# ncarraz/ESRGANplus

Measured on AMD Instinct MI355X. Metric: HR megapixels/sec (x4 SR) RRDBNet forward (fwd+bwd: the fwd_bwd object of this line), higher is better.
Workload: dtype f16; 1 GPU; RRDBNet x4 (23 RRDB, nf=64, gc=32) fp16 forward-only, batch 16 of 128x128 LR tiles per GPU -> 512x512 HR (BASELINE configs[1]); global_batch=16, parallelism=dp1 (independent tiles, no collective), weights=synthetic default-init seed 0

## Files before the change

### esrganplus_amd/_lib.py

```python
import ctypes as C
import os
import threading

import torch

_HERE = os.path.dirname(os.path.abspath(__file__))
LIB_PATH = os.environ.get('ESR_LIB_PATH', os.path.join(_HERE, 'libesrgan_hip.so'))

ESR_F16, ESR_F32 = 0, 1
ACT_NONE, ACT_LRELU, ACT_RELU = 0, 1, 2
NOISE_OFF, NOISE_PHILOX, NOISE_EXPLICIT = 0, 1, 2
OP_CONV, OP_PACK, OP_LAYOUT, OP_NOISE_FILL, OP_WGRAD, OP_BN, OP_POOL, OP_LINEAR, OP_UNPERMUTE, OP_PACK_BATCH = 1, 2, 3, 4, 5, 6, 7, 8, 9, 10
OP_RDB_CHAIN, OP_FRAG_GATHER, OP_RDB_WGRAD, OP_RDB_CHAIN_BWD = 11, 12, 13, 14
BN_STATS, BN_FINALIZE, BN_APPLY, BN_BWD_REDUCE, BN_BWD_FINAL, BN_BWD_APPLY, BN_RESTAT, BN_FIN_APPLY = 0, 1, 2, 3, 4, 5, 6, 7
NO_LAYER = 0xFFFFFFFF
POOL_FWD, POOL_BWD, POOL_SHUFFLE, POOL_UNSHUFFLE = 0, 1, 2, 3


class esr_g32(C.Structure):
    _fields_ = [('ptr', C.c_void_p), ('batch_stride', C.c_int64), ('group_stride', C.c_int64),
                ('wp', C.c_int32), ('ngroups', C.c_int32)]


class esr_conv(C.Structure):
    _fields_ = [('dtype', C.c_int32), ('ks', C.c_int32), ('stride', C.c_int32),
                ('upsample', C.c_int32), ('B', C.c_int32), ('H', C.c_int32), ('W', C.c_int32),
                ('cin_groups', C.c_int32), ('cout_blocks', C.c_int32),
                ('in_', esr_g32), ('out', esr_g32),
                ('w', C.c_void_p), ('bias', C.c_void_p), ('w1x1', C.c_void_p),
                ('n1x1_groups', C.c_int32), ('act', C.c_int32),
                ('aux_out', esr_g32),
                ('alpha', C.c_float), ('res1', esr_g32),
                ('beta', C.c_float), ('res2', esr_g32),
                ('noise_mode', C.c_int32), ('sigma', C.c_float), ('seed', C.c_uint64),
                ('layer1', C.c_uint32), ('layer2', C.c_uint32),
                ('z1', esr_g32), ('z2', esr_g32), ('mask', esr_g32), ('out2', esr_g32),
                ('nchw_out_c', C.c_int32), ('nchw_out', C.c_void_p),
                ('debug_flags', C.c_int32), ('mask_cb_begin', C.c_int32), ('gamma', C.c_float),
                ('layer3', C.c_uint32), ('z3', esr_g32), ('out3', esr_g32),
                ('mask_act', C.c_int32), ('_pad2', C.c_int32), ('seed_dev', C.c_void_p),
                ('ksplit', C.c_int32), ('stat_groups', C.c_int32), ('stat_C', C.c_int32), ('_pad3', C.c_int32),
                ('split_ws', C.c_void_p), ('stat_sums', C.c_void_p)]


class esr_pack(C.Structure):
    _fields_ = [('src', C.c_void_p), ('dst', C.c_void_p), ('cout', C.c_int32), ('cin', C.c_int32),
                ('ks', C.c_int32), ('dtype', C.c_int32), ('transpose_flip', C.c_int32),
                ('sum_dst', C.c_int32), ('sum_src', C.c_int32), ('sum_count', C.c_int32),
                ('ups_dgrad', C.c_int32),
                ('gather', C.c_int32), ('dst_cout', C.c_int32), ('dst_chunk0', C.c_int32),
                ('dst_nchunks', C.c_int32), ('src_co0', C.c_int32), ('src_ks', C.c_int32),
                ('scale', C.c_float), ('ups_fwd', C.c_int32), ('fold_co0', C.c_int32), ('one_t', C.c_int32)]


class esr_wgrad(C.Structure):
    _fields_ = [('dtype', C.c_int32), ('ks', C.c_int32), ('stride', C.c_int32),
                ('upsample', C.c_int32), ('B', C.c_int32), ('H', C.c_int32), ('W', C.c_int32),
                ('cout', C.c_int32), ('cin', C.c_int32), ('g', esr_g32), ('in_', esr_g32),
                ('dw', C.c_void_p), ('dbias', C.c_void_p), ('scale', C.c_float), ('tap_major', C.c_int32),
                ('partial', C.c_void_p), ('partial_elems', C.c_int64)]


class esr_layout(C.Structure):
    _fields_ = [('dtype', C.c_int32), ('to_g32', C.c_int32), ('B', C.c_int32), ('C', C.c_int32),
                ('H', C.c_int32), ('W', C.c_int32), ('nchw', C.c_void_p), ('g32', esr_g32),
                ('use_affine', C.c_int32), ('mean_c', C.c_float * 4), ('inv_std_c', C.c_float * 4),
                ('accumulate', C.c_int32), ('_pad', C.c_int32)]


class esr_noise_fill(C.Structure):
    _fields_ = [('dst', C.c_void_p), ('B', C.c_int32), ('C', C.c_int32), ('H', C.c_int32),
                ('W', C.c_int32), ('seed', C.c_uint64), ('layer', C.c_uint32)]


class esr_bn(C.Structure):
    _fields_ = [('dtype', C.c_int32), ('mode', C.c_int32), ('B', C.c_int32), ('C', C.c_int32),
                ('H', C.c_int32), ('W', C.c_int32), ('training', C.c_int32), ('act', C.c_int32),
                ('momentum', C.c_float), ('eps', C.c_float),
                ('x', esr_g32), ('y', esr_g32), ('g', esr_g32), ('gx', esr_g32),
                ('sums', C.c_void_p), ('mean', C.c_void_p), ('invstd', C.c_void_p),
                ('gamma', C.c_void_p), ('beta', C.c_void_p), ('running_mean', C.c_void_p),
                ('running_var', C.c_void_p), ('dgamma', C.c_void_p), ('dbeta', C.c_void_p),
                ('groups', C.c_int32), ('_pad', C.c_int32), ('num_batches_tracked', C.c_void_p)]


class esr_pool(C.Structure):
    _fields_ = [('dtype', C.c_int32), ('mode', C.c_int32), ('B', C.c_int32), ('C', C.c_int32),
                ('H', C.c_int32), ('W', C.c_int32), ('relu_mask', C.c_int32), ('_pad', C.c_int32),
                ('x', esr_g32), ('y', esr_g32), ('g', esr_g32), ('gx', esr_g32)]


class esr_linear(C.Structure):
    _fields_ = [('mode', C.c_int32), ('B', C.c_int32), ('I', C.c_int32), ('O', C.c_int32),
                ('act', C.c_int32), ('in_act', C.c_int32),
                ('x', C.c_void_p), ('w', C.c_void_p), ('b', C.c_void_p), ('y', C.c_void_p),
# ... 70 lines not shown
                ('band_rows', C.c_int32), ('band_margin', C.c_int32), ('img_H', C.c_int32), ('_pad3', C.c_int32)]


class esr_l1_loss(C.Structure):
    _fields_ = [('a', C.c_void_p), ('b', C.c_void_p), ('grad_a', C.c_void_p), ('loss', C.c_void_p),
                ('scratch', C.c_void_p), ('n', C.c_int64), ('weight', C.c_float), ('grad_scale', C.c_float),
                ('grad_scale_dev', C.c_void_p)]


class esr_ragan_loss(C.Structure):
    _fields_ = [('x', C.c_void_p), ('y', C.c_void_p), ('grad_x', C.c_void_p), ('grad_y', C.c_void_p),
                ('loss', C.c_void_p), ('mean_x', C.c_void_p), ('mean_y', C.c_void_p),
                ('bce_x', C.c_void_p), ('bce_y', C.c_void_p), ('n', C.c_int32),
                ('tx', C.c_float), ('ty', C.c_float), ('weight', C.c_float),
                ('mode', C.c_int32), ('grad_scale', C.c_float), ('sums', C.c_void_p), ('ext', C.c_void_p),
                ('grad_scale_dev', C.c_void_p)]


class esr_img_metrics(C.Structure):
    _fields_ = [('sr', C.c_void_p), ('hr', C.c_void_p), ('C', C.c_int32), ('H', C.c_int32), ('W', C.c_int32),
                ('crop', C.c_int32), ('y_only', C.c_int32), ('_pad', C.c_int32), ('lo', C.c_float), ('hi', C.c_float),
                ('img_sr', C.c_void_p), ('img_hr', C.c_void_p), ('y_sr', C.c_void_p), ('y_hr', C.c_void_p),
                ('out', C.c_void_p), ('win', C.c_double * 11)]


class esr_frag_gather(C.Structure):
    _fields_ = [('src_off', C.c_void_p), ('src_base', C.c_void_p), ('dst', C.c_void_p), ('n', C.c_int64),
                ('piece_bytes', C.c_int32), ('_pad', C.c_int32)]


class esr_rdb_wgrad_block(C.Structure):
    _fields_ = [('in_', esr_g32), ('q', esr_g32), ('dw', C.c_void_p * 6), ('db', C.c_void_p * 6)]


class esr_rdb_wgrad(C.Structure):
    _fields_ = [('dtype', C.c_int32), ('B', C.c_int32), ('H', C.c_int32), ('W', C.c_int32),
                ('n_blocks', C.c_int32), ('tap_major', C.c_int32), ('scale5', C.c_float), ('scale', C.c_float),
                ('blocks', C.c_void_p), ('partial', C.c_void_p), ('partial_elems', C.c_int64),
                ('max_workgroups', C.c_int32), ('_pad', C.c_int32)]


class _op_union(C.Union):
    _fields_ = [('conv', esr_conv), ('pack', esr_pack), ('layout', esr_layout),
                ('noise_fill', esr_noise_fill), ('wgrad', esr_wgrad), ('bn', esr_bn),
                ('pool', esr_pool), ('linear', esr_linear), ('unpermute', esr_unpermute),
                ('pack_batch', esr_pack_batch), ('rdb_chain', esr_rdb_chain), ('frag_gather', esr_frag_gather),
                ('rdb_wgrad', esr_rdb_wgrad)]


class esr_op(C.Structure):
    _fields_ = [('kind', C.c_int32), ('flags', C.c_int32), ('u', _op_union)]


EXPORTS = ['esr_packed_weight_bytes', 'esr_g32_dims', 'esr_conv_forward', 'esr_pack_conv_weights',
           'esr_convert_layout', 'esr_fill_noise', 'esr_conv_wgrad', 'esr_conv_wgrad_multi', 'esr_batchnorm', 'esr_maxpool2',
           'esr_linear_op', 'esr_grad_unpermute', 'esr_adam_step', 'esr_amp_step', 'esr_resample_axis', 'esr_pack_conv_weights_batch', 'esr_pack_pieces',
           'esr_run_ops', 'esr_run_ops_timed', 'esr_graph_create', 'esr_graph_launch', 'esr_graph_destroy', 'esr_last_error',
           'esr_abi_version', 'esr_sizeof_op', 'esr_rdb_forward', 'esr_rdb_workspace_bytes', 'esr_rdb_weight_stream_bytes',
           'esr_rdb_max_tiles_per_image', 'esr_gather_fragments', 'esr_image_metrics', 'esr_wgrad_workspace_elems',
           'esr_l1_loss_forward', 'esr_ragan_loss_forward', 'esr_rdb_wgrad_run', 'esr_rdb_wgrad_workspace_elems', 'esr_rdb_backward',
           'esr_rdb_mask_bytes', 'esr_rdb_check_abort', 'esr_debug_hold_cus', 'esr_debug_device_alias', 'esr_debug_chain_order_waits',
           'esr_debug_mfma_probe', 'esr_debug_rdb_wgrad_follow']

_lib = None
_lock = threading.Lock()


class HipExtensionError(RuntimeError):
    pass


def lib():
    global _lib
    if _lib is not None:
        return _lib
    with _lock:
        if _lib is not None:
            return _lib
        if not os.path.exists(LIB_PATH):
            raise HipExtensionError(
                'esrganplus_amd: %s not found — build it with `python -c "import __graft_entry__ as g; '
                'g.build()"` (hipcc --offload-arch=gfx950). There is no CPU/eager fallback.' % LIB_PATH)
        L = C.CDLL(LIB_PATH)
        for name in EXPORTS:
            if not hasattr(L, name):
                raise HipExtensionError('libesrgan_hip.so lacks symbol ' + name)
        L.esr_last_error.restype = C.c_char_p
        L.esr_sizeof_op.restype = C.c_size_t
        L.esr_pack_pieces.restype = C.c_int64
        L.esr_pack_pieces.argtypes = [C.POINTER(esr_pack)]
        L.esr_packed_weight_bytes.restype = C.c_size_t
        L.esr_packed_weight_bytes.argtypes = [C.c_int32] * 4
        L.esr_g32_dims.restype = None
        L.esr_g32_dims.argtypes = [C.c_int32, C.c_int32, C.POINTER(C.c_int32), C.POINTER(C.c_int32)]
        L.esr_run_ops.argtypes = [C.c_void_p, C.c_int32, C.c_void_p]
        L.esr_run_ops_timed.argtypes = [C.c_void_p, C.c_int32, C.c_void_p, C.c_void_p]
        L.esr_graph_create.argtypes = [C.c_void_p, C.c_int32, C.POINTER(C.c_void_p)]
        L.esr_graph_launch.argtypes = [C.c_void_p, C.c_void_p]
        L.esr_graph_destroy.argtypes = [C.c_void_p]
        L.esr_conv_wgrad_multi.argtypes = [C.POINTER(esr_wgrad), C.c_int32, C.c_void_p]
        L.esr_wgrad_workspace_elems.restype = C.c_int64
        L.esr_wgrad_workspace_elems.argtypes = [C.c_void_p, C.c_int32]
        L.esr_rdb_workspace_bytes.restype = C.c_size_t
        L.esr_rdb_workspace_bytes.argtypes = [C.c_int32] * 3
        L.esr_rdb_weight_stream_bytes.restype = C.c_size_t
        L.esr_rdb_weight_stream_bytes.argtypes = [C.c_int32]
        L.esr_rdb_mask_bytes.restype = C.c_size_t
        L.esr_rdb_mask_bytes.argtypes = [C.c_int32] * 3
        L.esr_debug_chain_order_waits.restype = C.c_uint64
        L.esr_debug_device_alias.argtypes = [C.c_int32]
        L.esr_rdb_wgrad_workspace_elems.restype = C.c_int64
        L.esr_rdb_wgrad_workspace_elems.argtypes = [C.c_int32] * 4
        for name, st in (('esr_conv_forward', esr_conv), ('esr_pack_conv_weights', esr_pack),
                         ('esr_convert_layout', esr_layout), ('esr_fill_noise', esr_noise_fill),
                         ('esr_conv_wgrad', esr_wgrad), ('esr_batchnorm', esr_bn),
                         ('esr_maxpool2', esr_pool), ('esr_linear_op', esr_linear),
                         ('esr_grad_unpermute', esr_unpermute), ('esr_adam_step', esr_adam), ('esr_amp_step', esr_amp), ('esr_resample_axis', esr_resample),
                         ('esr_pack_conv_weights_batch', esr_pack_batch), ('esr_rdb_forward', esr_rdb_chain),
                         ('esr_gather_fragments', esr_frag_gather), ('esr_image_metrics', esr_img_metrics),
                         ('esr_l1_loss_forward', esr_l1_loss), ('esr_ragan_loss_forward', esr_ragan_loss),
                         ('esr_rdb_wgrad_run', esr_rdb_wgrad), ('esr_rdb_backward', esr_rdb_chain)):
            getattr(L, name).argtypes = [C.POINTER(st), C.c_void_p]
        if L.esr_sizeof_op() != C.sizeof(esr_op):
            raise HipExtensionError('ABI mismatch: sizeof(esr_op) C=%d ctypes=%d'
                                    % (L.esr_sizeof_op(), C.sizeof(esr_op)))
        _lib = L
    return _lib


def check(rc, what=''):
    if rc != 0:
        raise HipExtensionError('%s failed (%d): %s' % (what or 'libesrgan_hip', rc,
                                                        lib().esr_last_error().decode()))


def g32_dims(h, w):
    hp, wp = C.c_int32(), C.c_int32()
    lib().esr_g32_dims(h, w, C.byref(hp), C.byref(wp))
    return hp.value, wp.value


def packed_weight_bytes(cout, cin, ks, dtype):
    return lib().esr_packed_weight_bytes(cout, cin, ks, dtype)


OPF_SIDE = 1
OPF_FOLLOW = 4
OPF_SIDE_FREE = 2


class OpList:

    def __init__(self):
        self.ops = []
        self._arr = None
        self.keep = []

    def add_conv(self, conv):
        o = esr_op()
        o.kind = OP_CONV
        o.u.conv = conv
        self.ops.append(o)
        self._arr = None
        self.drop_graph()
        return len(self.ops) - 1

# ... 73 lines not shown
```

### esrganplus_amd/csrc/api.hip

```cpp
#include <stdarg.h>
#include <stdio.h>
#include <stdlib.h>
#include <mutex>

#include "common.h"

namespace {
thread_local char g_err[512] = "";
}

void esr_set_error(const char* fmt, ...) {
  va_list ap;
  va_start(ap, fmt);
  vsnprintf(g_err, sizeof(g_err), fmt, ap);
  va_end(ap);
}

int esr_check_launch(const char* what) {
  const hipError_t e = hipGetLastError();
  if (e != hipSuccess) {
    esr_set_error("%s: %s", what, hipGetErrorString(e));
    return ESR_ERR_LAUNCH;
  }
  return ESR_OK;
// ... 21 lines not shown
namespace {
constexpr int NFREE = 3;
struct SideState { std::mutex mu; hipStream_t owner; hipStream_t stream; hipEvent_t fork[2], join[2]; hipStream_t xs[NFREE]; hipEvent_t xfork, xjoin[NFREE]; SideState* next; };
SideState* side_state(hipStream_t owner) {
  static std::mutex mu;
  static SideState* per_dev[64] = {};
  const int dev = esr_bookkeeping_device();
  static const bool per_stream = [] { const char* e = getenv("ESR_SIDE_PER_STREAM"); return e && atoi(e) != 0; }();
  if (!per_stream) owner = nullptr;
  std::lock_guard<std::mutex> lk(mu);
  for (SideState* s = per_dev[dev]; s; s = s->next)
    if (s->owner == owner) return s;
  SideState* s = new SideState();
  s->owner = owner;
  bool ok = hipStreamCreateWithFlags(&s->stream, hipStreamNonBlocking) == hipSuccess;
  for (int k = 0; k < 2 && ok; ++k)
    ok = hipEventCreateWithFlags(&s->fork[k], hipEventDisableTiming) == hipSuccess &&
         hipEventCreateWithFlags(&s->join[k], hipEventDisableTiming) == hipSuccess;
  ok = ok && hipEventCreateWithFlags(&s->xfork, hipEventDisableTiming) == hipSuccess;
  for (int k = 0; k < NFREE && ok; ++k)
    ok = hipStreamCreateWithFlags(&s->xs[k], hipStreamNonBlocking) == hipSuccess &&
         hipEventCreateWithFlags(&s->xjoin[k], hipEventDisableTiming) == hipSuccess;
  if (!ok) { esr_set_error("side stream: creation failed"); delete s; return nullptr; }
  s->next = per_dev[dev];
  per_dev[dev] = s;
  return s;
}
}

int esr_rdb_backward_with_follower(const esr_rdb_chain* ch, const esr_rdb_wgrad* wg, hipStream_t stream, hipStream_t side, hipEvent_t fork);

constexpr int ESR_WGRAD_RUN_MAX = 24;

extern "C" int esr_run_ops(const esr_op* ops, int32_t n, esr_stream_t stream) {
  if (!ops || n < 0) { esr_set_error("esr_run_ops: invalid arguments"); return ESR_ERR_INVALID; }
  if (esr_rdb_check_abort()) {
    esr_set_error("esr_run_ops: an earlier fused-chain launch aborted (a tile waited > 1 s for its neighbours: CUs held by other work?) — its results are invalid");
    return ESR_ERR_LAUNCH;
  }
  int nside = 0;
  bool joined = true;
  int nfree = 0;
  auto join_free = [&]() -> int {
    if (nfree > 0) {
      SideState* ss = side_state((hipStream_t)stream);
      for (int q = 0; q < NFREE && q < nfree; ++q) ESR_HIP(hipStreamWaitEvent((hipStream_t)stream, ss->xjoin[q], 0));
      nfree = 0;
    }
    return ESR_OK;
  };
  for (int i = 0; i < n; ++i) {
    int rc;
    switch (ops[i].kind) {
      case ESR_OP_CONV: rc = esr_conv_forward(&ops[i].u.conv, stream); break;
      case ESR_OP_PACK: rc = esr_pack_conv_weights(&ops[i].u.pack, stream); break;
      case ESR_OP_LAYOUT: rc = esr_convert_layout(&ops[i].u.layout, stream); break;
      case ESR_OP_NOISE_FILL: rc = esr_fill_noise(&ops[i].u.noise_fill, stream); break;
      case ESR_OP_WGRAD: {
        const int side = ops[i].flags & ESR_OPF_SIDE;
        int m = 1;
        while (i + m < n && m < ESR_WGRAD_RUN_MAX && ops[i + m].kind == ESR_OP_WGRAD && (ops[i + m].flags & ESR_OPF_SIDE) == side) ++m;
        esr_wgrad run[ESR_WGRAD_RUN_MAX];
        for (int k = 0; k < m; ++k) run[k] = ops[i + k].u.wgrad;
        if (!side) {
          rc = m == 1 ? esr_conv_wgrad(&run[0], stream) : esr_conv_wgrad_multi(run, m, stream);
        } else if (ops[i].flags & ESR_OPF_SIDE_FREE) {
          SideState* ss = side_state((hipStream_t)stream);
          if (!ss) return ESR_ERR_LAUNCH;
          const int q = nfree % NFREE;
          {
            std::lock_guard<std::mutex> lk(ss->mu);
            ESR_HIP(hipEventRecord(ss->xfork, (hipStream_t)stream));
            ESR_HIP(hipStreamWaitEvent(ss->xs[q], ss->xfork, 0));
          }
          rc = esr_conv_wgrad_multi(run, m, (esr_stream_t)ss->xs[q]);
          ESR_HIP(hipEventRecord(ss->xjoin[q], ss->xs[q]));
          ++nfree;
        } else {
          SideState* ss = side_state((hipStream_t)stream);
          if (!ss) return ESR_ERR_LAUNCH;
          hipStream_t main_st = (hipStream_t)stream;
          if (nside > 0) ESR_HIP(hipStreamWaitEvent(main_st, ss->join[(nside - 1) & 1], 0));
          {
            std::lock_guard<std::mutex> lk(ss->mu);
            ESR_HIP(hipEventRecord(ss->fork[nside & 1], main_st));
            ESR_HIP(hipStreamWaitEvent(ss->stream, ss->fork[nside & 1], 0));
          }
          rc = esr_conv_wgrad_multi(run, m, (esr_stream_t)ss->stream);
          ESR_HIP(hipEventRecord(ss->join[nside & 1], ss->stream));
          ++nside;
          joined = false;
        }
        if (rc == ESR_OK) i += m - 1;
        break;
      }
      case ESR_OP_BN: rc = esr_batchnorm(&ops[i].u.bn, stream); break;
      case ESR_OP_POOL: rc = esr_maxpool2(&ops[i].u.pool, stream); break;
      case ESR_OP_LINEAR: rc = esr_linear_op(&ops[i].u.linear, stream); break;
      case ESR_OP_UNPERMUTE:
        if ((rc = join_free()) != ESR_OK) break;
        if (nside > 0 && !joined) { ESR_HIP(hipStreamWaitEvent((hipStream_t)stream, side_state((hipStream_t)stream)->join[(nside - 1) & 1], 0)); joined = true; }
        rc = esr_grad_unpermute(&ops[i].u.unpermute, stream);
        break;
      case ESR_OP_PACK_BATCH: rc = esr_pack_conv_weights_batch(&ops[i].u.pack_batch, stream); break;
      case ESR_OP_RDB_CHAIN: rc = esr_rdb_forward(&ops[i].u.rdb_chain, stream); break;
      case ESR_OP_RDB_CHAIN_BWD: {
        if (i + 1 < n && ops[i + 1].kind == ESR_OP_RDB_WGRAD && (ops[i + 1].flags & ESR_OPF_FOLLOW)) {
// ... 158 lines not shown
```

### esrganplus_amd/engine.py

```python
import ctypes as C

import os

import torch

from . import _lib as L

SIGMA = 0.1

_STORE_FLAVOUR = int(os.environ.get('ESR_STORE_FLAVOUR', '0'))


def _dt(dtype):
    if dtype in ('fp16', torch.float16, L.ESR_F16):
        return L.ESR_F16, torch.float16, 16
    if dtype in ('fp32', torch.float32, L.ESR_F32):
        return L.ESR_F32, torch.float32, 8
    raise ValueError('dtype must be fp16 or fp32, got %r' % (dtype,))


def require_cuda(t, what):
    if not t.is_cuda:
        raise L.HipExtensionError(
            'esrganplus_amd: %s is on %s — the HIP path needs a CUDA/HIP tensor on an MI355X; '
# ... 250 lines not shown
                    for c in range(ks):
                        for kw in range(3):
                            offs += [frag(blk, c0 + c, kh, kw) for blk in range(ph, 6) for kh in range(3)]
                else:
                    for c in range(ks):
                        for kw in range(3):
                            offs += [frag(blk, c0 + c, kh, kw) for blk in (4, 5) for kh in range(3)]
        assert len(offs) * 1024 == len(self.prefixes) * self.stream_bytes, (len(offs), self.stream_bytes)
        return offs

    def ensure(self, stream, force=False):
        if self.ops is None:
            self._tab = torch.tensor(self._table(), dtype=torch.int64, device=self.arena.device)
            g = L.esr_frag_gather()
            g.src_off, g.src_base, g.dst, g.n = (self._tab.data_ptr(), self.dp.arena.data_ptr(),
                                                 self.arena.data_ptr(), self._tab.numel())
            self.ops = L.OpList()
            self.ops.add(L.OP_FRAG_GATHER, 'frag_gather', g)
        gen = getattr(self.dp, 'pack_count', 0)
        if force or gen != self._gen:
            self.ops.run(stream)
            self._gen = gen


def use_train_chain(dtype_e, B, H, W, explicit_z):
    if dtype_e != L.ESR_F16 or explicit_z or os.environ.get('ESR_RDB_TRAIN_CHAIN', '1') == '0':
        return False
    return rdb_chain_ok(B, H, W, False, False)


def rdb_chain_ok(B, H, W, noise, explicit_z):
    if os.environ.get('ESR_RDB_FUSED', '1') == '0' or (noise and explicit_z):
        return False
    tpi = ((H + 15) // 16) * ((W + 31) // 32)
    return tpi <= L.lib().esr_rdb_max_tiles_per_image()


def use_rdb_bands(dtype_e, H, W):
    mode = os.environ.get('ESR_RDB_BANDS', 'auto')
    if mode == '0' or os.environ.get('ESR_RDB_FUSED', '1') == '0' or rdb_band_geometry(H, W) is None:
        return False
    return mode == '1' or dtype_e == L.ESR_F16


def rdb_band_geometry(H, W):
    margin = 16
    tiles_x = (W + 31) // 32
    t = L.lib().esr_rdb_max_tiles_per_image() // tiles_x - 2 * (margin // 16)
    if t < 1:
        return None
    n = (H + 16 * t - 1) // (16 * t)
    rows = ((H + n - 1) // n + 15) // 16 * 16
    return rows, margin, n


def _conv(dtype_e, B, H, W, src, src_ch, dst, cw, act=L.ACT_NONE, ks=None, stride=1, upsample=0):
    c = L.esr_conv()
    c.dtype = dtype_e
    c.ks = cw.ks if ks is None else ks
    c.stride = stride
    c.upsample = upsample
    if upsample == 1 and getattr(cw, 'subpix', False):
        c.ks, c.upsample = 2, 3
    c.B, c.H, c.W = B, H, W
    cpg = 16 if dtype_e == L.ESR_F16 else 8
    c.cin_groups = (src_ch + cpg - 1) // cpg
    c.cout_blocks = (cw.cout + 31) // 32
    c.in_ = src
    if dst is not None:
        c.out = dst
    c.w = cw.w_ptr
    c.bias = cw.bias_ptr
    c.act = act
    c.alpha = 1.0
    c.beta = 1.0
    c.sigma = SIGMA
    c.noise_mode = L.NOISE_OFF
    c.layer1 = L.NO_LAYER
    c.layer2 = L.NO_LAYER
    c.layer3 = L.NO_LAYER
    c.gamma = 1.0
    c.mask_act = L.ACT_LRELU
    c.debug_flags = (_STORE_FLAVOUR << 3) | (int(os.environ.get('ESR_DBG', '0')) & ~7)
    return c


class Plan:

    def __init__(self):
        self.ops = L.OpList()
        self.bufs = []
        self.in_op = None
        self.out_op = None
        self.out_shape = None
        self.noise_ops = []
        self.chain_ops = []
        self.streams = None
        self.z_ops = []
        self.wgen = None
        self.chain_noise = False

    def run(self, x, out, stream, seed=0, zs=None):
        arr = self.ops.array()
        arr[self.in_op].u.layout.nchw = x.data_ptr()
        o = arr[self.out_op]
        if o.kind == L.OP_CONV:
# ... 202 lines not shown
    def n_noise_layers(self, nb):
        return (4 if self.variant == 'test_image' else 3) * nb if self.noise else 0

    def rrdbnet(self, nb, in_nc, out_nc, explicit_z):
        e = self.wp.entries
        B, H, W, d = self.B, self.H, self.W, self.dt_e
        P = self.plan
        self.zbufs = []
        if explicit_z and self.noise:
            self.alloc_z(self.n_noise_layers(nb))
        xin = self.buf(in_nc)
        fea = self.buf(64)
        P.in_op = self.import_nchw(xin, in_nc)
        if nb and rdb_chain_ok(B, H, W, self.noise, explicit_z):
            xa, xb = self.buf(64), self.buf(64)
            c = _conv(d, B, H, W, xin.view(0), in_nc, xa.view(0, 64), e['model.0'])
            c.aux_out = fea.view(0, 64)
            P.ops.add_conv(c)
            specs = []
            for i in range(nb):
                pre = 'model.1.sub.%d' % i
                specs.append((pre + '.RDB1', xa, xb, None, False))
                specs.append((pre + '.RDB2', xb, xb, None, False))
                specs.append((pre + '.RDB3', xb, xa, xa, self.variant == 'test_image'))
            self.rdb_chain(specs)
            x0, x1 = xa, xb
        elif nb and not self.noise and use_rdb_bands(self.dt_e, H, W):
            def head(dst):
                c = _conv(d, B, H, W, xin.view(0), in_nc, dst, e['model.0'])
                c.aux_out = fea.view(0, 64)
                P.ops.add_conv(c)
            res, x1 = self.rdb_chain_banded(nb, rdb_band_geometry(H, W), head), self.buf(64)
            c = _conv(d, B, H, W, res, 64, x1.view(0, 64), e['model.1.sub.%d' % nb])
            c.res1, c.alpha = fea.view(0, 64), 1.0
            P.ops.add_conv(c)
            x0 = None
        else:
            x0, x1, x2 = self.buf(192), self.buf(192), self.buf(192)
            c = _conv(d, B, H, W, xin.view(0), in_nc, x0.view(0, 64), e['model.0'])
            c.aux_out = fea.view(0, 64)
            P.ops.add_conv(c)
            for i in range(nb):
                self.rrdb('model.1.sub.%d' % i, x0, x1, x2)
        if x0 is not None:
            c = _conv(d, B, H, W, x0.view(0), 64, x1.view(0, 64), e['model.1.sub.%d' % nb])
            c.res1, c.alpha = fea.view(0, 64), 1.0
            P.ops.add_conv(c)
        u1 = self.buf(64, 2 * H, 2 * W)
        P.ops.add_conv(_conv(d, B, 2 * H, 2 * W, x1.view(0), 64, u1.view(0, 64), e['model.3'],
                             L.ACT_LRELU, upsample=1))
        u2 = self.buf(64, 4 * H, 4 * W)
        P.ops.add_conv(_conv(d, B, 4 * H, 4 * W, u1.view(0), 64, u2.view(0, 64), e['model.6'],
                             L.ACT_LRELU, upsample=1))
        u3 = self.buf(64, 4 * H, 4 * W)
        P.ops.add_conv(_conv(d, B, 4 * H, 4 * W, u2.view(0), 64, u3.view(0, 64), e['model.8'],
                             L.ACT_LRELU))
        c = _conv(d, B, 4 * H, 4 * W, u3.view(0), 64, None, e['model.10'])
        c.nchw_out_c = out_nc
        P.out_op = P.ops.add_conv(c)
        P.out_shape = (B, out_nc, 4 * H, 4 * W)
        return P


def use_graphs():
    return os.environ.get('ESR_GRAPH', '0') == '1'


def deterministic_wgrad():
    return os.environ.get('ESR_WGRAD_DET', '1') != '0'


def attach_wgrad_arena(oplist, device, exclusive=False):
    if not deterministic_wgrad():
        return None
    wops = [o for o in oplist.ops if o.kind == L.OP_WGRAD]
    if not wops:
        return None
    if exclusive:
        arr = oplist.array()
        needs = []
        for i, o in enumerate(oplist.ops):
            if o.kind == L.OP_WGRAD:
                n = L.lib().esr_wgrad_workspace_elems(C.cast(C.byref(arr[i]), C.c_void_p), 1)
                needs.append((o, (int(n) + 63) // 64 * 64))
        total = sum(n for _, n in needs)
        if total <= 0:
            return None
        arena = torch.empty(total, dtype=torch.float32, device=device)
        off = 0
        for o, n in needs:
            o.u.wgrad.partial, o.u.wgrad.partial_elems = (arena.data_ptr() + 4 * off, n) if n else (None, 0)
            off += n
        oplist._arr = None
        return arena
    need = L.lib().esr_wgrad_workspace_elems(C.cast(oplist.array(), C.c_void_p), len(oplist.ops))
    if need <= 0:
        return None
    arena = torch.empty(need, dtype=torch.float32, device=device)
    for o in wops:
        o.u.wgrad.partial, o.u.wgrad.partial_elems = arena.data_ptr(), need
    oplist._arr = None
    return arena


def attach_free_wgrad_regions(oplist, device):
    if not deterministic_wgrad():
        return None
    arr = oplist.array()
    needs = []
    for i, o in enumerate(oplist.ops):
# ... 846 lines not shown
```

### include/esrgan_hip.h

```cpp
#ifndef ESRGAN_HIP_H
#define ESRGAN_HIP_H

#include <stddef.h>
#include <stdint.h>

#ifdef __cplusplus
extern "C" {
#endif

typedef void* esr_stream_t;

enum esr_status {
  ESR_OK = 0,
  ESR_ERR_INVALID = -1,
  ESR_ERR_LAUNCH = -2,
  ESR_ERR_UNSUPPORTED = -3
};

enum esr_dtype { ESR_F16 = 0, ESR_F32 = 1 };
enum esr_act { ESR_ACT_NONE = 0, ESR_ACT_LRELU = 1 , ESR_ACT_RELU = 2 };
enum esr_noise { ESR_NOISE_OFF = 0, ESR_NOISE_PHILOX = 1, ESR_NOISE_EXPLICIT = 2 };

typedef struct esr_g32 {
  void* ptr;
  int64_t batch_stride;
  int64_t group_stride;
  int32_t wp;
  int32_t ngroups;
} esr_g32;

typedef struct esr_conv {
  int32_t dtype;
  int32_t ks;
  int32_t stride;
  int32_t upsample;
  int32_t B, H, W;
  int32_t cin_groups;
  int32_t cout_blocks;
  esr_g32 in;
  esr_g32 out;
  const void* w;
  const float* bias;
  const void* w1x1;
  int32_t n1x1_groups;
  int32_t act;
  esr_g32 aux_out;
  float alpha; esr_g32 res1;
  float beta;  esr_g32 res2;
  int32_t noise_mode;
  float sigma;
  uint64_t seed;
  uint32_t layer1, layer2;
  esr_g32 z1, z2;
  esr_g32 mask;
  esr_g32 out2;
  int32_t nchw_out_c;
  float* nchw_out;
  int32_t debug_flags;
  int32_t mask_cb_begin;
  float gamma;
  uint32_t layer3;
  esr_g32 z3;
  esr_g32 out3;
  int32_t mask_act;
  int32_t _pad2;
  const uint64_t* seed_dev;
  int32_t ksplit, stat_groups, stat_C, _pad3;
  float* split_ws;
  double* stat_sums;
} esr_conv;

typedef struct esr_pack {
  const float* src;
  void* dst;
  int32_t cout, cin, ks;
  int32_t dtype;
  int32_t transpose_flip;
  int32_t sum_dst;
  int32_t sum_src;
  int32_t sum_count;
  int32_t ups_dgrad;
  int32_t gather, dst_cout, dst_chunk0, dst_nchunks, src_co0, src_ks;
  float scale;
  int32_t ups_fwd;
  int32_t fold_co0;
  int32_t one_t;
} esr_pack;

typedef struct esr_pack_batch {
  const esr_pack* table;
  const int64_t* piece_begin;
  int32_t n, _pad;
  int64_t total_pieces;
} esr_pack_batch;
int64_t esr_pack_pieces(const esr_pack* p);

size_t esr_packed_weight_bytes(int32_t cout, int32_t cin, int32_t ks, int32_t dtype);

typedef struct esr_layout {
  int32_t dtype;
  int32_t to_g32;
  int32_t B, C, H, W;
  float* nchw;
  esr_g32 g32;
  int32_t use_affine;
  float mean_c[4];
  float inv_std_c[4];
  int32_t accumulate;
  int32_t _pad;
} esr_layout;

typedef struct esr_noise_fill {
  float* dst; int32_t B, C, H, W; uint64_t seed; uint32_t layer;
} esr_noise_fill;

typedef struct esr_wgrad {
  int32_t dtype, ks, stride, upsample;
  int32_t B, H, W;
  int32_t cout, cin;
  esr_g32 g;
  esr_g32 in;
  float* dw;
// ... 174 lines not shown
typedef struct esr_rdb_wgrad_block {
  esr_g32 in;
  esr_g32 q;
  float* dw[6];
  float* db[6];
} esr_rdb_wgrad_block;
typedef struct esr_rdb_wgrad {
  int32_t dtype;
  int32_t B, H, W;
  int32_t n_blocks, tap_major;
  float scale5;
  float scale;
  const esr_rdb_wgrad_block* blocks;
  float* partial;
  int64_t partial_elems;
  int32_t max_workgroups;
  int32_t _pad;
} esr_rdb_wgrad;

enum esr_op_kind { ESR_OP_CONV = 1, ESR_OP_PACK = 2, ESR_OP_LAYOUT = 3, ESR_OP_NOISE_FILL = 4,
                   ESR_OP_WGRAD = 5, ESR_OP_BN = 6, ESR_OP_POOL = 7, ESR_OP_LINEAR = 8,
                   ESR_OP_UNPERMUTE = 9, ESR_OP_PACK_BATCH = 10,
                   ESR_OP_RDB_CHAIN = 11, ESR_OP_FRAG_GATHER = 12, ESR_OP_RDB_WGRAD = 13,
                   ESR_OP_RDB_CHAIN_BWD = 14  };

#define ESR_OPF_SIDE 1
#define ESR_OPF_SIDE_FREE 2

#define ESR_OPF_FOLLOW 4

typedef struct esr_op {
  int32_t kind;
  int32_t flags;
  union {
    esr_conv conv;
    esr_pack pack;
    esr_layout layout;
    esr_noise_fill noise_fill;
    esr_wgrad wgrad;
    esr_bn bn;
    esr_pool pool;
    esr_linear linear;
    esr_unpermute unpermute;
    esr_pack_batch pack_batch;
    esr_rdb_chain rdb_chain;
    esr_frag_gather frag_gather;
    esr_rdb_wgrad rdb_wgrad;
  } u;
} esr_op;

void esr_g32_dims(int32_t H, int32_t W, int32_t* Hp, int32_t* Wp);

int esr_conv_forward(const esr_conv* p, esr_stream_t stream);
int esr_pack_conv_weights(const esr_pack* p, esr_stream_t stream);
int esr_convert_layout(const esr_layout* p, esr_stream_t stream);
int esr_fill_noise(const esr_noise_fill* p, esr_stream_t stream);
int esr_conv_wgrad(const esr_wgrad* p, esr_stream_t stream);
int esr_conv_wgrad_multi(const esr_wgrad* items, int32_t n, esr_stream_t stream);
int esr_batchnorm(const esr_bn* p, esr_stream_t stream);
int esr_maxpool2(const esr_pool* p, esr_stream_t stream);
int esr_linear_op(const esr_linear* p, esr_stream_t stream);
int esr_grad_unpermute(const esr_unpermute* p, esr_stream_t stream);
int esr_adam_step(const esr_adam* p, esr_stream_t stream);
int esr_amp_step(const esr_amp* p, esr_stream_t stream);
int esr_resample_axis(const esr_resample* p, esr_stream_t stream);
int esr_pack_conv_weights_batch(const esr_pack_batch* p, esr_stream_t stream);
int esr_rdb_forward(const esr_rdb_chain* p, esr_stream_t stream);
int esr_rdb_backward(const esr_rdb_chain* p, esr_stream_t stream);
size_t esr_rdb_mask_bytes(int32_t B, int32_t H, int32_t W);
int esr_rdb_check_abort(void);
int esr_debug_hold_cus(int32_t n_workgroups, const uint32_t* release, uint32_t max_ms, uint32_t* started, esr_stream_t stream);
int esr_debug_mfma_probe(const void* operands, int32_t iters, uint64_t* clk2, float* sink, int32_t n_workgroups, esr_stream_t stream);
int esr_debug_rdb_wgrad_follow(const struct esr_rdb_wgrad* p, const uint32_t* flags, int32_t tiles_x, int32_t tiles_y, esr_stream_t stream);
int esr_debug_device_alias(int32_t alias);
uint64_t esr_debug_chain_order_waits(void);
size_t esr_rdb_workspace_bytes(int32_t B, int32_t H, int32_t W);
size_t esr_rdb_weight_stream_bytes(int32_t dtype);
int esr_rdb_max_tiles_per_image(void);
int esr_gather_fragments(const esr_frag_gather* g, esr_stream_t stream);
int esr_rdb_wgrad_run(const esr_rdb_wgrad* p, esr_stream_t stream);
int64_t esr_rdb_wgrad_workspace_elems(int32_t B, int32_t H, int32_t W, int32_t n_blocks);
int esr_image_metrics(const esr_img_metrics* p, esr_stream_t stream);

int esr_l1_loss_forward(const esr_l1_loss* p, esr_stream_t stream);
int esr_ragan_loss_forward(const esr_ragan_loss* p, esr_stream_t stream);

int esr_run_ops(const esr_op* ops, int32_t n, esr_stream_t stream);
int64_t esr_wgrad_workspace_elems(const esr_op* ops, int32_t n);

typedef struct esr_graph_s* esr_graph_t;
int esr_graph_create(const esr_op* ops, int32_t n, esr_graph_t* out);
int esr_graph_launch(esr_graph_t g, esr_stream_t stream);
int esr_graph_destroy(esr_graph_t g);

int esr_run_ops_timed(const esr_op* ops, int32_t n, esr_stream_t stream, float* ms_out);

const char* esr_last_error(void);
int esr_abi_version(void);
size_t esr_sizeof_op(void);

#ifdef __cplusplus
}
#endif
#endif
```

Measured before the change: 500.1 HR-Mpix/s.

## Fuse the last two HR 3x3 convs into one tiled kernel

Adds a kernel that computes the 64->64 LeakyReLU conv (model.8) over a haloed tile, keeps that intermediate in LDS, then runs the final 64->out_nc conv (model.10) from LDS and writes NCHW fp32 output directly. This removes the full-resolution 64-channel intermediate buffer write and re-read at 512x512 HR, which is a large memory-traffic cost. In exchange it recomputes halo rows and columns of the first conv per tile and introduces new LDS and tiling logic. It is enabled by default through an environment flag and falls back to the old path when shapes don't match.

```diff
diff --git a/esrganplus_amd/_lib.py b/esrganplus_amd/_lib.py
--- a/esrganplus_amd/_lib.py
+++ b/esrganplus_amd/_lib.py
@@ -40,7 +40,8 @@
                 ('layer3', C.c_uint32), ('z3', esr_g32), ('out3', esr_g32),
                 ('mask_act', C.c_int32), ('_pad2', C.c_int32), ('seed_dev', C.c_void_p),
                 ('ksplit', C.c_int32), ('stat_groups', C.c_int32), ('stat_C', C.c_int32), ('_pad3', C.c_int32),
-                ('split_ws', C.c_void_p), ('stat_sums', C.c_void_p)]
+                ('split_ws', C.c_void_p), ('stat_sums', C.c_void_p),
+                ('w2', C.c_void_p), ('bias2', C.c_void_p), ('cout2', C.c_int32), ('_pad4', C.c_int32)]
 
 
 class esr_pack(C.Structure):
@@ -217,7 +218,7 @@
     _fields_ = [('kind', C.c_int32), ('flags', C.c_int32), ('u', _op_union)]
 
 
-EXPORTS = ['esr_packed_weight_bytes', 'esr_g32_dims', 'esr_conv_forward', 'esr_pack_conv_weights',
+EXPORTS = ['esr_packed_weight_bytes', 'esr_g32_dims', 'esr_conv_forward', 'esr_conv_pair_forward', 'esr_pack_conv_weights',
            'esr_convert_layout', 'esr_fill_noise', 'esr_conv_wgrad', 'esr_conv_wgrad_multi', 'esr_batchnorm', 'esr_maxpool2',
            'esr_linear_op', 'esr_grad_unpermute', 'esr_adam_step', 'esr_amp_step', 'esr_resample_axis', 'esr_pack_conv_weights_batch', 'esr_pack_pieces',
            'esr_run_ops', 'esr_run_ops_timed', 'esr_graph_create', 'esr_graph_launch', 'esr_graph_destroy', 'esr_last_error',
@@ -276,7 +277,7 @@
         L.esr_debug_device_alias.argtypes = [C.c_int32]
         L.esr_rdb_wgrad_workspace_elems.restype = C.c_int64
         L.esr_rdb_wgrad_workspace_elems.argtypes = [C.c_int32] * 4
-        for name, st in (('esr_conv_forward', esr_conv), ('esr_pack_conv_weights', esr_pack),
+        for name, st in (('esr_conv_forward', esr_conv), ('esr_conv_pair_forward', esr_conv), ('esr_pack_conv_weights', esr_pack),
                          ('esr_convert_layout', esr_layout), ('esr_fill_noise', esr_noise_fill),
                          ('esr_conv_wgrad', esr_wgrad), ('esr_batchnorm', esr_bn),
                          ('esr_maxpool2', esr_pool), ('esr_linear_op', esr_linear),
diff --git a/esrganplus_amd/csrc/api.hip b/esrganplus_amd/csrc/api.hip
--- a/esrganplus_amd/csrc/api.hip
+++ b/esrganplus_amd/csrc/api.hip
@@ -97,7 +97,7 @@
   for (int i = 0; i < n; ++i) {
     int rc;
     switch (ops[i].kind) {
-      case ESR_OP_CONV: rc = esr_conv_forward(&ops[i].u.conv, stream); break;
+      case ESR_OP_CONV: rc = ops[i].u.conv.w2 ? esr_conv_pair_forward(&ops[i].u.conv, stream) : esr_conv_forward(&ops[i].u.conv, stream); break;
       case ESR_OP_PACK: rc = esr_pack_conv_weights(&ops[i].u.pack, stream); break;
       case ESR_OP_LAYOUT: rc = esr_convert_layout(&ops[i].u.layout, stream); break;
       case ESR_OP_NOISE_FILL: rc = esr_fill_noise(&ops[i].u.noise_fill, stream); break;
diff --git a/esrganplus_amd/csrc/hr_tail_fused.hip b/esrganplus_amd/csrc/hr_tail_fused.hip
--- /dev/null
+++ b/esrganplus_amd/csrc/hr_tail_fused.hip
@@ -0,0 +1,260 @@
+#include "common.h"
+#include "mfma_tile.h"
+
+namespace {
+
+typedef __attribute__((ext_vector_type(4))) float f32x4_t;
+
+struct HG {
+  static constexpr int NW = 4, NT = NW * 64;
+  static constexpr int MH = 16, MW = 32;
+  static constexpr int OH = MH - 2, OW = MW - 2;
+  static constexpr int IH = MH + 2, IW = MW + 2;
+  static constexpr int R = 4;
+  static constexpr int WIH = R + 2;
+  static constexpr int NSLOT = IH * IW * 2;
+  static constexpr int NLD = (NSLOT + NT - 1) / NT;
+  static constexpr int ACT = NLD * NT * 16;
+  static constexpr int NCW = 2, NTAP = 9;
+  static constexpr int WWIN = NCW * NTAP;
+  static constexpr int WLD = (WWIN + NW - 1) / NW;
+  static constexpr int WBYTES = WWIN * 1024;
+  static constexpr int WOFF = 2 * ACT;
+  static constexpr int MID = 8 * MH * MW * 16;
+  static constexpr int LDS_BYTES = 2 * ACT + 2 * WBYTES;
+  static constexpr int ROWS2 = OH / 2;
+  static_assert(MID <= LDS_BYTES, "the intermediate tile overlays the K loop's stages");
+  static_assert(LDS_BYTES <= 80 * 1024, "two workgroups per CU");
+};
+
+__device__ __forceinline__ void mma16(f32x4_t& acc, const u32x4& a, const u32x4& b) {
+  acc = __builtin_amdgcn_mfma_f32_16x16x32_f16(__builtin_bit_cast(half8, a), __builtin_bit_cast(half8, b), acc, 0, 0, 0);
+}
+
+__global__ __launch_bounds__(HG::NT, 2) void hr_tail_fused_kernel(const esr_conv p) {
+  using G = HG;
+  __shared__ __attribute__((aligned(16))) char smem[G::LDS_BYTES];
+  constexpr int R = G::R, NCW = G::NCW;
+  const int tid = threadIdx.x;
+  const int lane = tid & 63;
+  const int wave = __builtin_amdgcn_readfirstlane(tid >> 6);
+  const int wr = wave;
+  const int j = lane & 31, h = lane >> 5;
+
+  const int tiles_x = (p.W + G::OW - 1) / G::OW, tiles_y = (p.H + G::OH - 1) / G::OH;
+  int t;
+  {
+    const int nwg = gridDim.x, bid = blockIdx.x, xcd = bid & 7, q = nwg >> 3, r = nwg & 7;
+    t = (xcd < r ? xcd * (q + 1) : r * (q + 1) + (xcd - r) * q) + (bid >> 3);
+  }
+  const int tx = t % tiles_x, ty = (t / tiles_x) % tiles_y, b = t / (tiles_x * tiles_y);
+  const int oy0 = ty * G::OH, ox0 = tx * G::OW;
+
+  const int iy0 = oy0 - 1, ix0 = ox0 - 1;
+  int goff[G::NLD];
+#pragma unroll
+  for (int i = 0; i < G::NLD; ++i) {
+    int s = tid + G::NT * i;
+    if (s >= G::NSLOT) s = G::NSLOT - 1;
+    const int row = s / (2 * G::IW), rem = s - row * 2 * G::IW;
+    const int col = rem >> 1, hs = rem & 1, half = hs ^ ((col >> 3) & 1);
+    int prow = iy0 + row, pcol = ix0 + col;
+    if (prow < 0 || prow > p.H + 1 || pcol < 0 || pcol > p.W + 1) { prow = 0; pcol = 0; }
+    goff[i] = (prow * p.in.wp + pcol) * 32 + half * 16;
+  }
+  const char* const in_b = (const char*)p.in.ptr + b * p.in.batch_stride;
+  const int64_t in_gs = p.in.group_stride;
+  char* const lds_wv = smem + wave * 1024;
+
+  int colofs[3];
+#pragma unroll
+  for (int kw = 0; kw < 3; ++kw) {
+    const int col = j + kw;
+    colofs[kw] = col * 32 + ((h ^ ((col >> 3) & 1)) << 4) + wr * R * G::IW * 32;
+  }
+
+  constexpr int NCHUNK = 4;
+  const char* wsrc[G::WLD];
+  int wdst[G::WLD];
+#pragma unroll
+  for (int i = 0; i < G::WLD; ++i) {
+    const int q = (wave + G::NW * i) % G::WWIN;
+    const int blk = q / G::NTAP;
+    wdst[i] = q * 1024;
+    wsrc[i] = (const char*)p.w + (int64_t)blk * NCHUNK * G::NTAP * 1024 + ((q - blk * G::NTAP) * 64 + lane) * 16;
+  }
+
+  Acc8 acc;
+  acc_zero(acc);
+
+  auto stage_acts = [&](int chunk, int sa) __attribute__((always_inline)) {
+    const char* src = in_b + (int64_t)chunk * in_gs;
+    char* dst = lds_wv + sa * G::ACT;
+#pragma unroll
+    for (int i = 0; i < G::NLD; ++i) dma16_act(src + goff[i], dst + G::NT * 16 * i);
+  };
+  auto stage_wts = [&](int chunk, int sw) __attribute__((always_inline)) {
+#pragma unroll
+    for (int i = 0; i < G::WLD; ++i) dma16(wsrc[i] + chunk * (G::NTAP * 1024), smem + G::WOFF + sw * G::WBYTES + wdst[i]);
+  };
+
+  stage_wts(0, 0);
+  stage_acts(0, 0);
+  for (int c = 0; c < NCHUNK; ++c) {
+    asm volatile("s_waitcnt vmcnt(0)" ::: "memory");
+    __builtin_amdgcn_s_barrier();
+    if (c + 1 < NCHUNK) {
+      stage_wts(c + 1, (c + 1) & 1);
+      stage_acts(c + 1, (c + 1) & 1);
+    }
+    const char* lds = smem + (c & 1) * G::ACT;
+    const char* ldw = smem + G::WOFF + (c & 1) * G::WBYTES + lane * 16;
+
+    u32x4 af[2][3 * NCW], bf[2][G::WIH];
+    auto read_step = [&](auto KW, u32x4 (&a)[3 * NCW], u32x4 (&bq)[G::WIH]) __attribute__((always_inline)) {
+      constexpr int kw = decltype(KW)::value;
+#pragma unroll
+      for (int kh = 0; kh < 3; ++kh)
+#pragma unroll
+        for (int cw = 0; cw < NCW; ++cw) a[kh * NCW + cw] = *(const u32x4*)(ldw + (cw * G::NTAP + kh * 3 + kw) * 1024);
+#pragma unroll
+      for (int ir = 0; ir < G::WIH; ++ir) bq[ir] = *(const u32x4*)(lds + colofs[kw] + ir * G::IW * 32);
+    };
+    read_step(std::integral_constant<int, 0>{}, af[0], bf[0]);
+    sfor<3>([&](auto KW) __attribute__((always_inline)) {
+      constexpr int kw = decltype(KW)::value;
+      constexpr int cur = kw & 1;
+      if constexpr (kw + 1 < 3) read_step(std::integral_constant<int, kw + 1>{}, af[cur ^ 1], bf[cur ^ 1]);
+      sfor<G::WIH>([&](auto IR) __attribute__((always_inline)) {
+        constexpr int ir = decltype(IR)::value;
+        sfor<3>([&](auto KH) __attribute__((always_inline)) {
+          constexpr int kh = decltype(KH)::value;
+          constexpr int r = ir - kh;
+          if constexpr (r >= 0 && r < R) {
+            sfor<NCW>([&](auto CW) __attribute__((always_inline)) {
+              constexpr int cw = decltype(CW)::value;
+              mma<_Float16>(accsel<r * NCW + cw>(acc), af[cur][kh * NCW + cw], bf[cur][ir]);
+            });
+          }
+        });
+      });
+    });
+  }
+
+  __syncthreads();
+
+  {
+    const int gx = ox0 - 1 + j;
+    const bool col_in = gx >= 0 && gx < p.W;
+    sfor<NCW>([&](auto CW) __attribute__((always_inline)) {
+      constexpr int cw = decltype(CW)::value;
+      f32x4 bq[4];
+#pragma unroll
+      for (int i = 0; i < 4; ++i) bq[i] = p.bias ? *(const f32x4*)(p.bias + cw * 32 + 16 * h + 4 * i) : f32x4{0.f, 0.f, 0.f, 0.f};
+      sfor<R>([&](auto RR) __attribute__((always_inline)) {
+        constexpr int r = decltype(RR)::value;
+        const int my = wr * R + r, gy = oy0 - 1 + my;
+        const bool inside = col_in && gy >= 0 && gy < p.H;
+        const f32x16 a = accsel<r * NCW + cw>(acc);
+        half8 x, y;
+#pragma unroll
+        for (int e = 0; e < 16; ++e) {
+          const float s = a[e] + bq[e >> 2][e & 3];
+          const float v = inside ? fmaxf(s, s * ESR_LRELU_SLOPE) : 0.f;
+          if (e < 8) x[e] = (_Float16)v; else y[e - 8] = (_Float16)v;
+        }
+        const int u0 = cw * 4 + 2 * h;
+        *(u32x4*)(smem + (((u0 * G::MH + my) * G::MW) + j) * 16) = __builtin_bit_cast(u32x4, x);
+        *(u32x4*)(smem + ((((u0 + 1) * G::MH + my) * G::MW) + j) * 16) = __builtin_bit_cast(u32x4, y);
+      });
+    });
+  }
+  const int n = lane & 15, kb = lane >> 4;
+  u32x4 a2[2][G::NTAP];
+  {
+    const int i2 = (n >> 2) + 8 * (n & 3);
+#pragma unroll
+    for (int kc = 0; kc < 2; ++kc)
+#pragma unroll
+      for (int tp = 0; tp < G::NTAP; ++tp)
+        a2[kc][tp] = *(const u32x4*)((const char*)p.w2 + (((2 * kc + (kb >> 1)) * G::NTAP + tp) * 64 + i2 + 32 * (kb & 1)) * 16);
+  }
+
+  __syncthreads();
+
+  const int cgp = wave & 1, rg = wave >> 1;
+  const int cs = cgp * (G::OW - 16), r0 = rg * G::ROWS2;
+  f32x4_t o0 = {0.f, 0.f, 0.f, 0.f}, o1 = o0, o2 = o0, o3 = o0, o4 = o0, o5 = o0, o6 = o0;
+  auto osel = [&](auto RR) __attribute__((always_inline)) -> f32x4_t& {
+    constexpr int r = decltype(RR)::value;
+    if constexpr (r == 0) return o0;
+    else if constexpr (r == 1) return o1;
+    else if constexpr (r == 2) return o2;
+    else if constexpr (r == 3) return o3;
+    else if constexpr (r == 4) return o4;
+    else if constexpr (r == 5) return o5;
+    else return o6;
+  };
+  const char* const mid = smem + ((kb * G::MH + r0) * G::MW + cs + n) * 16;
+  sfor<G::ROWS2 + 2>([&](auto IR) __attribute__((always_inline)) {
+    constexpr int ir = decltype(IR)::value;
+    sfor<3>([&](auto KW) __attribute__((always_inline)) {
+      constexpr int kw = decltype(KW)::value;
+      sfor<2>([&](auto KC) __attribute__((always_inline)) {
+        constexpr int kc = decltype(KC)::value;
+        const u32x4 bfr = *(const u32x4*)(mid + ((kc * 4 * G::MH + ir) * G::MW + kw) * 16);
+        sfor<3>([&](auto KH) __attribute__((always_inline)) {
+          constexpr int kh = decltype(KH)::value;
+          constexpr int r = ir - kh;
+          if constexpr (r >= 0 && r < G::ROWS2) mma16(osel(std::integral_constant<int, r>{}), a2[kc][kh * 3 + kw], bfr);
+        });
+      });
+    });
+  });
+
+  const int ox = ox0 + cs + n;
+  if (ox >= p.W || (cgp && n < 16 - (G::OW - 16))) return;
+  float b2[4];
+#pragma unroll
+  for (int i = 0; i < 4; ++i) b2[i] = (p.bias2 && 4 * i + kb < p.cout2) ? p.bias2[4 * i + kb] : 0.f;
+  const int64_t plane = (int64_t)p.H * p.W;
+  float* const ob = p.nchw_out + ((int64_t)b * p.cout2 + kb) * plane + ox;
+  sfor<G::ROWS2>([&](auto RR) __attribute__((always_inline)) {
+    constexpr int r = decltype(RR)::value;
+    const int oy = oy0 + r0 + r;
+    if (oy >= p.H) return;
+    const f32x4_t v = osel(RR);
+#pragma unroll
+    for (int i = 0; i < 4; ++i)
+      if (4 * i + kb < p.cout2) ob[(int64_t)(4 * i) * plane + (int64_t)oy * p.W] = v[i] + b2[i];
+  });
+}
+
+}
+
+extern "C" int esr_conv_pair_forward(const esr_conv* p, esr_stream_t stream) {
+  if (!p || !p->in.ptr || !p->w || !p->w2 || !p->nchw_out || p->B <= 0 || p->H <= 0 || p->W <= 0) {
+    esr_set_error("esr_conv_pair_forward: invalid arguments");
+    return ESR_ERR_INVALID;
+  }
+  if (p->dtype != ESR_F16) { esr_set_error("esr_conv_pair_forward: fp16 only (dtype %d)", p->dtype); return ESR_ERR_UNSUPPORTED; }
+  if (p->ks != 3 || p->stride != 1 || p->upsample) {
+    esr_set_error("esr_conv_pair_forward: both layers are 3x3/s1 (ks=%d stride=%d upsample=%d)", p->ks, p->stride, p->upsample);
+    return ESR_ERR_UNSUPPORTED;
+  }
+  if (p->cin_groups != 4 || p->in.ngroups < 4) { esr_set_error("esr_conv_pair_forward: 64 input channels only (cin_groups=%d)", p->cin_groups); return ESR_ERR_UNSUPPORTED; }
+  if (p->cout_blocks != 2) { esr_set_error("esr_conv_pair_forward: 64 mid channels only (cout_blocks=%d)", p->cout_blocks); return ESR_ERR_UNSUPPORTED; }
+  if (p->cout2 <= 0 || p->cout2 > 16) { esr_set_error("esr_conv_pair_forward: 1..16 output channels (cout2=%d)", p->cout2); return ESR_ERR_UNSUPPORTED; }
+  if (p->nchw_out_c != p->cout2) { esr_set_error("esr_conv_pair_forward: nchw_out_c (%d) must equal cout2 (%d)", p->nchw_out_c, p->cout2); return ESR_ERR_INVALID; }
+  if (p->act != ESR_ACT_LRELU) { esr_set_error("esr_conv_pair_forward: the first layer's activation is LeakyReLU (act=%d)", p->act); return ESR_ERR_UNSUPPORTED; }
+  if (p->out.ptr || p->aux_out.ptr || p->w1x1 || p->res1.ptr || p->res2.ptr || p->mask.ptr || p->out2.ptr || p->out3.ptr ||
+      p->noise_mode != ESR_NOISE_OFF || p->alpha != 1.0f || p->ksplit > 1 || p->stat_sums) {
+    esr_set_error("esr_conv_pair_forward: bias + activation only (no G32 output, residual, noise, 1x1, mask or split-K stage)");
+    return ESR_ERR_UNSUPPORTED;
+  }
+  if ((int64_t)(p->H + 2) * p->in.wp * 32 >= (int64_t)1 << 31) { esr_set_error("esr_conv_pair_forward: one channel-group plane must be < 2 GB"); return ESR_ERR_UNSUPPORTED; }
+  const int64_t tiles = (int64_t)((p->W + HG::OW - 1) / HG::OW) * ((p->H + HG::OH - 1) / HG::OH) * p->B;
+  if (tiles >= (int64_t)1 << 31) { esr_set_error("esr_conv_pair_forward: grid too large"); return ESR_ERR_UNSUPPORTED; }
+  hipLaunchKernelGGL(hr_tail_fused_kernel, dim3((unsigned)tiles), dim3(HG::NT), 0, (hipStream_t)stream, *p);
+  return esr_check_launch("hr_tail_fused_kernel");
+}
diff --git a/esrganplus_amd/engine.py b/esrganplus_amd/engine.py
--- a/esrganplus_amd/engine.py
+++ b/esrganplus_amd/engine.py
@@ -326,6 +326,11 @@
     n = (H + 16 * t - 1) // (16 * t)
     rows = ((H + n - 1) // n + 15) // 16 * 16
     return rows, margin, n
+
+
+def fused_hr_tail(dtype_e, c0, c1):
+    return (dtype_e == L.ESR_F16 and os.environ.get('ESR_FUSED_HR_TAIL', '1') != '0' and
+            (c0.cout, c0.cin, c0.ks) == (64, 64, 3) and c1.cin == 64 and c1.ks == 3 and c1.cout <= 16)
 
 
 def _conv(dtype_e, B, H, W, src, src_ch, dst, cw, act=L.ACT_NONE, ks=None, stride=1, upsample=0):
@@ -634,10 +639,14 @@
         u2 = self.buf(64, 4 * H, 4 * W)
         P.ops.add_conv(_conv(d, B, 4 * H, 4 * W, u1.view(0), 64, u2.view(0, 64), e['model.6'],
                              L.ACT_LRELU, upsample=1))
-        u3 = self.buf(64, 4 * H, 4 * W)
-        P.ops.add_conv(_conv(d, B, 4 * H, 4 * W, u2.view(0), 64, u3.view(0, 64), e['model.8'],
-                             L.ACT_LRELU))
-        c = _conv(d, B, 4 * H, 4 * W, u3.view(0), 64, None, e['model.10'])
+        if fused_hr_tail(d, e['model.8'], e['model.10']):
+            c = _conv(d, B, 4 * H, 4 * W, u2.view(0), 64, None, e['model.8'], L.ACT_LRELU)
+            c.w2, c.bias2, c.cout2 = e['model.10'].w_ptr, e['model.10'].bias_ptr, out_nc
+        else:
+            u3 = self.buf(64, 4 * H, 4 * W)
+            P.ops.add_conv(_conv(d, B, 4 * H, 4 * W, u2.view(0), 64, u3.view(0, 64), e['model.8'],
+                                 L.ACT_LRELU))
+            c = _conv(d, B, 4 * H, 4 * W, u3.view(0), 64, None, e['model.10'])
         c.nchw_out_c = out_nc
         P.out_op = P.ops.add_conv(c)
         P.out_shape = (B, out_nc, 4 * H, 4 * W)
diff --git a/include/esrgan_hip.h b/include/esrgan_hip.h
--- a/include/esrgan_hip.h
+++ b/include/esrgan_hip.h
@@ -68,6 +68,9 @@
   int32_t ksplit, stat_groups, stat_C, _pad3;
   float* split_ws;
   double* stat_sums;
+  const void* w2;
+  const float* bias2;
+  int32_t cout2, _pad4;
 } esr_conv;
 
 typedef struct esr_pack {
@@ -348,6 +351,7 @@
 void esr_g32_dims(int32_t H, int32_t W, int32_t* Hp, int32_t* Wp);
 
 int esr_conv_forward(const esr_conv* p, esr_stream_t stream);
+int esr_conv_pair_forward(const esr_conv* p, esr_stream_t stream);
 int esr_pack_conv_weights(const esr_pack* p, esr_stream_t stream);
 int esr_convert_layout(const esr_layout* p, esr_stream_t stream);
 int esr_fill_noise(const esr_noise_fill* p, esr_stream_t stream);
```

After: 500.9 HR-Mpix/s, median of 2. About the same (+0.2%).
